# treangenlab/komb

Measured on AMD Instinct MI355X. Metric: peeled edges/sec (k-truss), higher is better.
Workload: dtype int32

## Files before the change

komb_amd/api.py:

```python
import ctypes
import os

import numpy as np

from . import _lib
from ._lib import KombOpts, KombStats, as_c, ptr


class KombError(RuntimeError):
    def __init__(self, code, msg):
        super().__init__(f"komb_accel error {code}: {msg}")
        self.code = code


def gen_hug_edges(nv, n_cliques, alpha=2.6, seed=42):
    lib = _lib.load()
    n_raw = lib.komb_gen_hug_edges(nv, n_cliques, alpha, seed, None)
    if n_raw < 0:
        raise ValueError("komb_gen_hug_edges: bad arguments")
    uv = np.empty((n_raw, 2), dtype=np.int64)
    got = lib.komb_gen_hug_edges(nv, n_cliques, alpha, seed, ptr(uv))
    assert got == n_raw
    return uv


FORWARD_ENV_OPTIONS = False
OPTION_NAMES = ("FINISH", "LOCAL_LIMIT", "LOCAL_ITEMS", "LOCAL_DENSITY", "LOCAL_DEFER_CHUNKS", "TAIL", "CORE_TAIL", "INDEX",
                "REC_CAP", "OWN_DENSE_CAP", "NO_OWN_DENSE", "NO_REC_SCRATCH", "NO_FIRST_QUEUE", "FULL_CAPS", "PREP_ROW_STAGE", "RETIRE_EVERY", "SHARD_ENGINE",
                "TRI_DEBUG", "POOL_DEBUG", "BUILD_DEBUG", "LOCAL_DEBUG", "TAIL_DEBUG", "COMP_SAMPLE", "COMM_SHORT", "COMM_HEAVY", "POISON")

SENTINEL_I32 = -0x5A5A5A5B


def _out_i32(n):
    return np.full(n, SENTINEL_I32, dtype=np.int32)


def _out_f64(n):
    return np.full(n, np.nan, dtype=np.float64)


class KombAccel:
    def __init__(self, device=0, verbosity=0, flags=0):
        self._lib = _lib.load()
        opts = KombOpts(device=device, verbosity=verbosity)
        opts.reserved[0] = flags
        self._ctx = self._lib.komb_create(ctypes.byref(opts))
        if not self._ctx:
            raise MemoryError("komb_create failed")
        self.device = device
        self.nv = -1
        self.ne = 0
        self._forwarded = {}

    def set_option(self, name, value):
        v = None if value is None else str(value).encode()
        self._check(self._lib.komb_set_option(self._ctx, name.encode(), v))

    def _sync_env_options(self):
        if not FORWARD_ENV_OPTIONS:
            return
        for name in OPTION_NAMES:
            v = os.environ.get("KOMB_" + name)
            if name == "INDEX" and os.environ.get("KOMB_TWO_PASS"):
                v = "two_pass"
            if name == "SHARD_ENGINE" and v is None:
                v = os.environ.get("KOMB_SHARD_PEEL")
            if self._forwarded.get(name) != v:
                self.set_option(name, v)
                self._forwarded[name] = v

    def close(self):
        if getattr(self, "_ctx", None):
            self._lib.komb_destroy(self._ctx)
            self._ctx = None

    def __del__(self):
        self.close()

    def __enter__(self):
        return self

    def __exit__(self, *a):
        self.close()

    def _check(self, rc):
        if rc != 0:
            raise KombError(rc, self._lib.komb_last_error(self._ctx).decode())

    def from_edges(self, nv, uv):
        uv = as_c(np.asarray(uv).reshape(-1, 2), np.int64)
        self._sync_env_options()
        self._check(self._lib.komb_graph_from_edges(self._ctx, nv, uv.shape[0], ptr(uv)))
        self._info()
        return self

    def from_csr(self, rowptr, col):
        rowptr = as_c(rowptr, np.int64)
        col = as_c(col, np.int32)
        self._sync_env_options()
        self._check(self._lib.komb_graph_from_csr(self._ctx, len(rowptr) - 1, ptr(rowptr), ptr(col)))
        self._info()
        return self

    def _info(self):
        nv, ne = ctypes.c_int64(), ctypes.c_int64()
        self._check(self._lib.komb_graph_info(self._ctx, ctypes.byref(nv), ctypes.byref(ne)))
        self.nv, self.ne = nv.value, ne.value

    def get_csr(self):
        rowptr = np.full(self.nv + 1, SENTINEL_I32, dtype=np.int64)
# ... 244 lines not shown
```

komb_amd/csrc/truss_prep.hip:

```cpp
#include "truss_line.h"

#include <algorithm>

namespace komb {

namespace {

constexpr uint32_t kPrepHeavy = 2048;
constexpr uint32_t kRowCap = 1024;
constexpr uint32_t kRowStage = 8192;
constexpr int kPW = kBlock / kWave;
constexpr int kPrepU = 4;

__global__ __launch_bounds__(kBlock) void k_prep_vertex(const uint32_t *__restrict__ rowptr, const int32_t *__restrict__ col, int64_t nv,
                                                        uint32_t *__restrict__ dkey, uint32_t *__restrict__ dval,
                                                        uint32_t *__restrict__ first_upper, uint32_t *__restrict__ upper_cnt)
{
    for (int64_t v = (int64_t)blockIdx.x * kBlock + threadIdx.x; v <= nv; v += (int64_t)gridDim.x * kBlock) {
        if (v == nv) { upper_cnt[v] = 0u; continue; }
        const uint32_t b = rowptr[v], e = rowptr[v + 1];
        dkey[v] = e - b;
        dval[v] = (uint32_t)v;
        uint32_t lo = b, hi = e;
        while (lo < hi) {
            const uint32_t mid = lo + ((hi - lo) >> 1);
            if (col[mid] < (int32_t)v) lo = mid + 1; else hi = mid;
        }
        first_upper[v] = lo;
        upper_cnt[v] = e - lo;
    }
}

__global__ __launch_bounds__(kBlock) void k_prep_invert(const uint32_t *__restrict__ sorted_ids, const uint32_t *__restrict__ sorted_deg,
                                                        const uint32_t *__restrict__ regbase, int64_t nv, int32_t *__restrict__ i2o, int32_t *__restrict__ o2i,
                                                        uint32_t *__restrict__ backcur, uint32_t *__restrict__ nlocal)
{
    for (int64_t i = (int64_t)blockIdx.x * kBlock + threadIdx.x; i < nv; i += (int64_t)gridDim.x * kBlock) {
        const uint32_t v = sorted_ids[i];
        i2o[i] = (int32_t)v;
        o2i[v] = (int32_t)i;
        const uint32_t r0 = regbase[i], d = sorted_deg[i];
        backcur[i] = r0 + d - 1u;
        if (d > kPrepHeavy) nlocal[v] = 0u;
    }
}

__device__ __forceinline__ int owner_of(const uint32_t *s_end, uint32_t it)
{
    int lo = 0;
#pragma unroll
    for (int st = kWave / 2; st > 0; st >>= 1) lo += (s_end[lo + st - 1] <= it) ? st : 0;
    return lo;
}

__global__ __launch_bounds__(kBlock) void k_prep_kept(const uint32_t *__restrict__ rowptr, const int32_t *__restrict__ col, int64_t nv,
                                                      const int32_t *__restrict__ o2i, const uint32_t *__restrict__ fu, const uint32_t *__restrict__ ebase,
                                                      const uint32_t *__restrict__ regbase,
                                                      uint2 *__restrict__ tmp, uint32_t *__restrict__ nlocal, uint32_t *__restrict__ backcur)
{
    __shared__ uint32_t sh_end[kPW][kWave], sh_beg[kPW][kWave], sh_a[kPW][kWave], sh_rp[kPW][kWave], sh_eb[kPW][kWave], sh_cnt[kPW][kWave];
    const int lane = lane_id(), w = (int)(threadIdx.x >> 6);
    uint32_t *s_end = sh_end[w], *s_beg = sh_beg[w], *s_a = sh_a[w], *s_rp = sh_rp[w], *s_eb = sh_eb[w], *s_cnt = sh_cnt[w];
    const int64_t gw = ((int64_t)blockIdx.x * kBlock + threadIdx.x) >> 6, nw = ((int64_t)gridDim.x * kBlock) >> 6;
    const int64_t ntasks = (nv + kWave - 1) / kWave;
    for (int64_t task = gw; task < ntasks; task += nw) {
        const int64_t v0 = task * kWave, v = v0 + lane;
        const bool has = v < nv;
        const uint32_t beg = has ? rowptr[v] : 0u, end = has ? rowptr[v + 1] : 0u, up = has ? fu[v] : 0u;
        const bool heavy = end - beg > kPrepHeavy;
        const uint32_t incl = wave_incl_scan(heavy ? 0u : end - up);
        const uint32_t total = (uint32_t)__shfl((int)incl, kWave - 1);
        __builtin_amdgcn_wave_barrier();
        s_end[lane] = incl;
        s_beg[lane] = up;
        const uint32_t av = has ? (uint32_t)o2i[v] : 0u;
        s_a[lane] = av;
        s_rp[lane] = has ? regbase[av] : 0u;
        s_eb[lane] = has ? ebase[v] : 0u;
        s_cnt[lane] = 0u;
        __builtin_amdgcn_wave_barrier();
        for (uint32_t it0 = 0; it0 < total; it0 += kWave * kPrepU) {
            int t[kPrepU];
            uint32_t rowstart[kPrepU], j[kPrepU], b[kPrepU];
            int32_t wv[kPrepU];
            bool on[kPrepU];
#pragma unroll
            for (int u = 0; u < kPrepU; ++u) {
                const uint32_t it = it0 + (uint32_t)(u * kWave + lane);
                on[u] = it < total;
                t[u] = on[u] ? owner_of(s_end, it) : 0;
                rowstart[u] = t[u] ? s_end[t[u] - 1] : 0u;
                j[u] = s_beg[t[u]] + (it - rowstart[u]);
            }
#pragma unroll
            for (int u = 0; u < kPrepU; ++u) wv[u] = on[u] ? col[j[u]] : 0;
#pragma unroll
            for (int u = 0; u < kPrepU; ++u) b[u] = on[u] ? (uint32_t)o2i[wv[u]] : 0u;
#pragma unroll
            for (int u = 0; u < kPrepU; ++u) {
                const uint32_t base = it0 + (uint32_t)(u * kWave), it = base + (uint32_t)lane;
                if (base >= total) break;
                const int tt = t[u];
                const uint32_t a = s_a[tt];
                const uint32_t k = s_eb[tt] + (it - rowstart[u]);
                const bool mine = on[u] && b[u] > a, theirs = on[u] && b[u] < a;
                if (theirs) tmp[atomicSub(&backcur[b[u]], 1u)] = make_uint2(a, k);
                const uint64_t K = __ballot(mine);
                const uint32_t f = rowstart[u] > base ? rowstart[u] - base : 0u;
                const uint32_t r = s_cnt[tt] + (uint32_t)__popcll(K & lanemask_lt() & ~((1ull << f) - 1ull));
                if (mine) tmp[(size_t)s_rp[tt] + r] = make_uint2(b[u], k);
                __builtin_amdgcn_wave_barrier();
                if (on[u] && (it + 1u == s_end[tt] || lane == kWave - 1)) s_cnt[tt] = r + (mine ? 1u : 0u);
                __builtin_amdgcn_wave_barrier();
            }
        }
        if (has && !heavy) nlocal[v] = s_cnt[lane];
        __builtin_amdgcn_wave_barrier();
    }
}

constexpr uint32_t kHeavyChunk = 256;
__global__ __launch_bounds__(kBlock) void k_prep_kept_heavy(const uint32_t *__restrict__ rowptr, const int32_t *__restrict__ col, int64_t nv,
                                                            const uint32_t *__restrict__ sorted_deg, const int32_t *__restrict__ i2o,
                                                            const int32_t *__restrict__ o2i, const uint32_t *__restrict__ fu, const uint32_t *__restrict__ ebase,
                                                            const uint32_t *__restrict__ regbase,
                                                            uint2 *__restrict__ tmp, uint32_t *__restrict__ nlocal, uint32_t *__restrict__ backcur)
{
    const int lane = lane_id();
    const uint32_t wi = (uint32_t)(((int64_t)blockIdx.x * kBlock + threadIdx.x) >> 6), W = (uint32_t)(((int64_t)gridDim.x * kBlock) >> 6);
    uint32_t cbase = 0;
    for (int64_t h0 = 0; h0 < nv; h0 += kWave) {
        const int64_t a = nv - 1 - h0 - lane;
        const uint32_t deg = a >= 0 ? sorted_deg[a] : 0u;
        const bool hv = deg > kPrepHeavy;
        const uint64_t HM = __ballot(hv);
        if (HM == 0) break;
        int32_t v = 0;
        uint32_t fuv = 0, eb = 0, reg = 0, end = 0;
        if (hv) { v = i2o[a]; fuv = fu[v]; eb = ebase[v]; reg = regbase[a]; end = rowptr[v] + deg; }
        const uint32_t nch = hv ? (end - fuv + kHeavyChunk - 1) / kHeavyChunk : 0u;
        uint32_t inc = nch;
#pragma unroll
        for (int d = 1; d < kWave; d <<= 1) { const uint32_t t = (uint32_t)__shfl_up((int)inc, d); if (lane >= d) inc += t; }
        const int nh = __popcll(HM);
        const uint32_t tot = (uint32_t)__shfl((int)inc, kWave - 1);
        for (uint32_t rel = (wi + W - (cbase % W)) % W; rel < tot; rel += W) {
            const int t = __popcll(__ballot(inc <= rel));
            const uint32_t c = rel - ((uint32_t)__shfl((int)inc, t) - (uint32_t)__shfl((int)nch, t));
            const int32_t rv = __shfl(v, t);
            const uint32_t ra = (uint32_t)(nv - 1 - h0 - t);
            const uint32_t r_fu = (uint32_t)__shfl((int)fuv, t), r_eb = (uint32_t)__shfl((int)eb, t), r_reg = (uint32_t)__shfl((int)reg, t), r_end = (uint32_t)__shfl((int)end, t);
            {
                const uint32_t j0 = r_fu + c * kHeavyChunk;
                constexpr int kU = (int)(kHeavyChunk / kWave);
                bool on[kU];
                int32_t wv[kU];
                uint32_t b[kU];
#pragma unroll
                for (int u = 0; u < kU; ++u) { const uint32_t j = j0 + (uint32_t)(u * kWave + lane); on[u] = j < r_end; wv[u] = on[u] ? col[j] : 0; }
#pragma unroll
                for (int u = 0; u < kU; ++u) b[u] = on[u] ? (uint32_t)o2i[wv[u]] : 0u;
#pragma unroll
                for (int u = 0; u < kU; ++u) {
                    const uint32_t k = r_eb + (j0 + (uint32_t)(u * kWave + lane) - r_fu);
                    const bool mine = on[u] && b[u] > ra, theirs = on[u] && b[u] < ra;
                    if (theirs) tmp[atomicSub(&backcur[b[u]], 1u)] = make_uint2(ra, k);
                    const uint64_t K = __ballot(mine);
                    if (K) {
                        const int lead = __ffsll((long long)K) - 1;
                        uint32_t base = 0;
                        if (lane == lead) base = atomicAdd(&nlocal[rv], (uint32_t)__popcll(K));
                        base = (uint32_t)__shfl((int)base, lead);
                        if (mine) tmp[(size_t)r_reg + base + (uint32_t)__popcll(K & lanemask_lt())] = make_uint2(b[u], k);
                    }
                }
            }
        }
        cbase += tot;
        if (nh < kWave) break;
    }
}

__global__ __launch_bounds__(kBlock) void k_prep_dplus(int64_t nv, const int32_t *__restrict__ i2o, const uint32_t *__restrict__ sorted_deg,
                                                       const uint32_t *__restrict__ regbase, const uint32_t *__restrict__ backcur,
                                                       const uint32_t *__restrict__ nlocal,
                                                       uint32_t *__restrict__ dplus_i, uint4 *__restrict__ where_i, unsigned long long *__restrict__ own_bound)
{
    unsigned long long ob = 0;
    for (int64_t a = (int64_t)blockIdx.x * kBlock + threadIdx.x; a < nv; a += (int64_t)gridDim.x * kBlock) {
        const uint32_t nl = nlocal[i2o[a]], bk = backcur[a] + 1u, reg = regbase[a];
        const unsigned long long d = nl + (reg + sorted_deg[a] - bk);
        dplus_i[a] = (uint32_t)d;
        where_i[a] = make_uint4(reg, nl, bk, 0u);
        ob += d ? d * (d - 1ull) : 0ull;
    }
    block_add_u64(ob, own_bound);
}

__global__ __launch_bounds__(kBlock) void k_prep_rows(const uint32_t *__restrict__ orow, int64_t nv, const uint4 *__restrict__ where_i,
                                                      const uint2 *__restrict__ tmp, int32_t *__restrict__ ocol,
                                                      uint32_t *__restrict__ e2k, uint4 *__restrict__ line)
{
    __shared__ int32_t sh_b[kPW][kRowCap];
    __shared__ uint32_t sh_kk[kPW][kRowCap];
    __shared__ unsigned long long sh_sig[kPW][kWave][kSigBlocks];
    __shared__ int32_t sh_piv[kPW][kWave][kPivots];
    __shared__ uint32_t sh_end[kPW][kWave], sh_rp[kPW][kWave], sh_ob[kPW][kWave], sh_nl[kPW][kWave], sh_bk[kPW][kWave];
    const int lane = lane_id(), w = (int)(threadIdx.x >> 6);
    int32_t *s_b = sh_b[w];
    uint32_t *s_kk = sh_kk[w], *s_end = sh_end[w], *s_rp = sh_rp[w], *s_ob = sh_ob[w], *s_nl = sh_nl[w], *s_bk = sh_bk[w];
    unsigned long long (*s_sig)[kSigBlocks] = sh_sig[w];
    int32_t (*s_piv)[kPivots] = sh_piv[w];
    const int64_t gw = ((int64_t)blockIdx.x * kBlock + threadIdx.x) >> 6, nw = ((int64_t)gridDim.x * kBlock) >> 6;
    const int64_t ntasks = (nv + kWave - 1) / kWave;
    for (int64_t task = gw; task < ntasks; task += nw) {
        const int64_t a0 = task * kWave, a = a0 + lane;
        const bool has = a < nv;
        const uint32_t ob = has ? orow[a] : 0u, d = has ? orow[a + 1] - ob : 0u;
        const bool big = d > kRowCap;
        const uint4 wh = has ? where_i[a] : make_uint4(0u, 0u, 0u, 0u);
        const uint32_t len = big ? 0u : d;
        __builtin_amdgcn_wave_barrier();
        s_rp[lane] = wh.x;
        s_nl[lane] = wh.y;
        s_bk[lane] = wh.z;
        s_ob[lane] = ob;
#pragma unroll
        for (int x = 0; x < kSigBlocks; ++x) s_sig[lane][x] = 0ull;
#pragma unroll
        for (int x = 0; x < kPivots; ++x) s_piv[lane][x] = 0x7FFFFFFF;
        for (int done = 0; done < kWave;) {
            const uint32_t incl = wave_incl_scan(lane >= done ? len : 0u);
            const int nfit = __popcll(__ballot(lane >= done && incl <= kRowCap));
            const int r1 = done + nfit;
            const uint32_t E = (uint32_t)__shfl((int)incl, r1 - 1);
            __builtin_amdgcn_wave_barrier();
            s_end[lane] = lane < done ? 0u : (lane < r1 ? incl : 0xFFFFFFFFu);
            __builtin_amdgcn_wave_barrier();
            for (uint32_t k = (uint32_t)lane; k < E; k += kWave) {
                const int t = owner_of(s_end, k);
                const uint32_t first = t ? s_end[t - 1] : 0u;
                const uint32_t idx = k - first, nl = s_nl[t];
                const uint2 ent = tmp[idx < nl ? (size_t)s_rp[t] + idx : (size_t)s_bk[t] + (idx - nl)];
                s_b[k] = (int32_t)ent.x; s_kk[k] = ent.y;
            }
            __builtin_amdgcn_wave_barrier();
            for (uint32_t k = (uint32_t)lane; k < E; k += kWave) {
                const int t = owner_of(s_end, k);
                const uint32_t first = t ? s_end[t - 1] : 0u, last = s_end[t];
                const int32_t mine = s_b[k];
                uint32_t rank = 0;
                for (uint32_t x = first; x < last; ++x) rank += s_b[x] < mine ? 1u : 0u;
                const uint32_t e = s_ob[t] + rank;
                ocol[e] = mine;
                e2k[e] = s_kk[k];
                uint32_t blk; unsigned long long mask;
                sig_slot(mine, blk, mask);
                atomicOr(&s_sig[t][blk], mask);
                const uint32_t seg = (last - first + (uint32_t)kPivots) / (uint32_t)(kPivots + 1);
                if (rank && rank % seg == 0u && rank / seg <= (uint32_t)kPivots) s_piv[t][rank / seg - 1u] = mine;
            }
            __builtin_amdgcn_wave_barrier();
            done = r1;
        }
        if (has && !big) {
            uint4 *L = line + 4 * a;
            const int32_t *pv = s_piv[lane];
            const unsigned long long *sg = s_sig[lane];
            L[0] = make_uint4(ob, d, (uint32_t)pv[0], (uint32_t)pv[1]);
            L[1] = make_uint4((uint32_t)pv[2], (uint32_t)pv[3], (uint32_t)pv[4], (uint32_t)pv[5]);
            L[2] = make_uint4((uint32_t)sg[0], (uint32_t)(sg[0] >> 32), (uint32_t)sg[1], (uint32_t)(sg[1] >> 32));
            L[3] = make_uint4((uint32_t)sg[2], (uint32_t)(sg[2] >> 32), (uint32_t)sg[3], (uint32_t)(sg[3] >> 32));
        }
        __builtin_amdgcn_wave_barrier();
// ... 142 lines not shown
            const uint32_t j = j0 + me;
            const int32_t wv = j < end ? col[j] : 0;
            const bool keep = j < end && mask[wv];
            const uint64_t K = __ballot(keep);
            uint32_t before = 0, all = (uint32_t)__popcll(K);
            if (WG) {
                __syncthreads();
                if (lane == 0) sh_wc[w] = all;
                __syncthreads();
                all = 0;
#pragma unroll
                for (int q = 0; q < kBlock / kWave; ++q) { const uint32_t c = sh_wc[q]; if (q < w) before += c; all += c; }
            }
            if (FILL && keep) sub_col[out0 + run + before + (uint32_t)__popcll(K & lanemask_lt())] = (int32_t)vnew[wv];
            run += all;
        }
        if (!FILL && me == 0) subdeg[x] = run;
    }
}

__global__ __launch_bounds__(kBlock) void k_edge_list(const uint32_t *__restrict__ rowptr, const int32_t *__restrict__ col, int64_t nv,
                                                      const uint32_t *__restrict__ fu, const uint32_t *__restrict__ ebase, const int32_t *__restrict__ vold,
                                                      int32_t *__restrict__ eu, int32_t *__restrict__ ev)
{
    const int lane = lane_id();
    const int64_t gw = ((int64_t)blockIdx.x * kBlock + threadIdx.x) >> 6, nw = ((int64_t)gridDim.x * kBlock) >> 6;
    for (int64_t v = gw; v < nv; v += nw) {
        const uint32_t j0 = fu[v], j1 = rowptr[v + 1], k0 = ebase[v];
        const int32_t uo = vold ? vold[v] : (int32_t)v;
        for (uint32_t j = j0 + (uint32_t)lane; j < j1; j += kWave) {
            const int32_t w = col[j];
            eu[k0 + (j - j0)] = uo;
            ev[k0 + (j - j0)] = vold ? vold[w] : w;
        }
    }
}

inline int id_bits(int64_t nv)
{
    int vb = 1;
    while (vb < 31 && (1ll << vb) < nv) ++vb;
    return vb;
}

template <class T> hipError_t pool_get(komb_ctx *ctx, T **out, size_t count)
{
    return ctx->pool.get((void **)out, (count ? count : 1) * sizeof(T));
}

}

void prep_free(komb_ctx *ctx, TrussPrep *p)
{
    void *all[] = {p->o2i, p->i2o, p->orow, p->ocol, p->osrc, p->e2k, p->vline, p->wtasks};
    for (void *q : all) ctx->pool.put(q);
    *p = TrussPrep{};
}

int prep_build(komb_ctx *ctx, const uint32_t *rowptr, const int32_t *col, int64_t nv, int64_t ns, TrussPrep *out)
{
    hipStream_t s = ctx->stream;
    const int64_t ne = ns / 2;
    Range r_all("truss: prepare");
    prep_free(ctx, out);
    TrussPrep P;
    P.nv = nv; P.ne = ne;
    struct Fail { komb_ctx *c; TrussPrep *p; bool armed = true; ~Fail() { if (armed) prep_free(c, p); } } fail{ctx, &P};
    EventSet evs;
    hipEvent_t ev[5] = {nullptr, nullptr, nullptr, nullptr, nullptr};
    for (auto &e : ev) KOMB_HIP(ctx, evs.make(&e));
    KOMB_HIP(ctx, hipEventRecord(ev[0], s));
    KOMB_HIP(ctx, pool_get(ctx, &P.o2i, (size_t)nv));
    KOMB_HIP(ctx, pool_get(ctx, &P.i2o, (size_t)nv));
    KOMB_HIP(ctx, pool_get(ctx, &P.orow, (size_t)nv + 1));
    KOMB_HIP(ctx, pool_get(ctx, &P.ocol, (size_t)ne + 8));
    KOMB_HIP(ctx, pool_get(ctx, &P.e2k, (size_t)ne));
    KOMB_HIP(ctx, pool_get(ctx, &P.vline, 4 * (size_t)nv));
    const size_t task_cap = 2 * (size_t)nv + (size_t)ne / kWave + 64;
    KOMB_HIP(ctx, pool_get(ctx, (uint2 **)&P.wtasks, task_cap));
    KOMB_HIP(ctx, hipMemsetAsync(P.ocol + ne, 0, 8 * sizeof(int32_t), s));

    DevBufs bufs(ctx);
    uint32_t *d_dk[2] = {nullptr, nullptr}, *d_dv[2] = {nullptr, nullptr}, *d_fu = nullptr, *d_uc = nullptr, *d_ebase = nullptr, *d_dplus = nullptr;
    uint32_t *d_nlocal = nullptr, *d_backcur = nullptr, *d_regbase = nullptr;
    uint4 *d_where = nullptr;
    uint32_t *d_tcnt = nullptr, *d_hlist = nullptr, *d_words = nullptr;
    unsigned long long *d_acc = nullptr;
    uint2 *d_tmp = nullptr;
    for (int i = 0; i < 2; ++i) { KOMB_HIP(ctx, bufs.alloc(&d_dk[i], (size_t)nv)); KOMB_HIP(ctx, bufs.alloc(&d_dv[i], (size_t)nv)); }
    KOMB_HIP(ctx, bufs.alloc(&d_fu, (size_t)nv + 1));
    KOMB_HIP(ctx, bufs.alloc(&d_uc, (size_t)nv + 1));
    KOMB_HIP(ctx, bufs.alloc(&d_ebase, (size_t)nv + 1));
    KOMB_HIP(ctx, bufs.alloc(&d_dplus, (size_t)nv + 1));
    KOMB_HIP(ctx, bufs.alloc(&d_nlocal, (size_t)nv));
    KOMB_HIP(ctx, bufs.alloc(&d_where, (size_t)nv));
    KOMB_HIP(ctx, bufs.alloc(&d_regbase, (size_t)nv + 1));
    KOMB_HIP(ctx, bufs.alloc(&d_backcur, (size_t)nv));
    KOMB_HIP(ctx, bufs.alloc(&d_tcnt, (size_t)nv + 1));
    const uint32_t hcap = (uint32_t)(ne / kRowCap + 64);
    KOMB_HIP(ctx, bufs.alloc(&d_hlist, (size_t)hcap));
    KOMB_HIP(ctx, bufs.alloc(&d_words, 4));
    KOMB_HIP(ctx, bufs.alloc(&d_acc, 8));
    KOMB_HIP(ctx, bufs.alloc(&d_tmp, (size_t)ns));
    KOMB_HIP(ctx, hipMemsetAsync(d_words, 0, 4 * sizeof(uint32_t), s));
    KOMB_HIP(ctx, hipMemsetAsync(d_acc, 0, 8 * sizeof(unsigned long long), s));
    KOMB_HIP(ctx, hipMemsetAsync(d_dplus + nv, 0, sizeof(uint32_t), s));

    const int gv = grid_for(nv + 1);
    const int gwave = grid_for((nv + kWave - 1) / kWave, kPW, 256 * 8);
    k_prep_vertex<<<gv, kBlock, 0, s>>>(rowptr, col, nv, d_dk[0], d_dv[0], d_fu, d_uc);
    uint32_t *sk = d_dk[0], *sv = d_dv[0];
    if (nv > 0) {
        KOMB_TRY(prim_sort_pairs_u32_u32(ctx, d_dk[0], d_dk[1], d_dv[0], d_dv[1], nv, id_bits(nv), &sk, &sv));
        KOMB_TRY(prim_exclusive_sum_u32(ctx, sk, d_regbase, nv));
        k_prep_invert<<<grid_for(nv), kBlock, 0, s>>>(sv, sk, d_regbase, nv, P.i2o, P.o2i, d_backcur, d_nlocal);
    }
    KOMB_TRY(prim_exclusive_sum_u32(ctx, d_uc, d_ebase, nv + 1));
    KOMB_HIP(ctx, hipEventRecord(ev[1], s));
    if (nv > 0) {
        k_prep_kept<<<gwave, kBlock, 0, s>>>(rowptr, col, nv, P.o2i, d_fu, d_ebase, d_regbase, d_tmp, d_nlocal, d_backcur);
        k_prep_kept_heavy<<<256 * 4, kBlock, 0, s>>>(rowptr, col, nv, sk, P.i2o, P.o2i, d_fu, d_ebase, d_regbase, d_tmp, d_nlocal, d_backcur);
        k_prep_dplus<<<grid_for(nv), kBlock, 0, s>>>(nv, P.i2o, sk, d_regbase, d_backcur, d_nlocal, d_dplus, d_where, d_acc);
    }
    KOMB_TRY(prim_exclusive_sum_u32(ctx, d_dplus, P.orow, nv + 1));
    KOMB_HIP(ctx, hipEventRecord(ev[2], s));
    const int group = (int)std::max<int64_t>(1, std::min<int64_t>(kWedgeV, nv / (256 * KOMB_WEDGE_EU * kTriWaves * 4)));
    k_task_count<<<gv, kBlock, 0, s>>>(P.orow, nv, group, d_tcnt, d_hlist, d_words, hcap);
    if (nv > 0) {
        k_prep_rows<<<gwave, kBlock, 0, s>>>(P.orow, nv, d_where, d_tmp, P.ocol, P.e2k, P.vline);
        uint32_t stage_cap = kRowStage;
        if (const char *e = ctx_opt(ctx, "PREP_ROW_STAGE")) stage_cap = std::min<uint32_t>(kRowStage, (uint32_t)strtoul(e, nullptr, 10));
        k_prep_rows_heavy<<<1024, kBlock, 0, s>>>(d_hlist, d_words, P.orow, d_where, d_tmp, P.ocol, P.e2k, P.vline, stage_cap);
    }
    KOMB_HIP(ctx, hipEventRecord(ev[3], s));
    KOMB_TRY(prim_exclusive_sum_u32(ctx, d_tcnt, d_tcnt, nv + 1));
    if (nv > 0) k_task_fill<<<grid_for(nv), kBlock, 0, s>>>(d_tcnt, nv, group, (uint2 *)P.wtasks);
    k_prep_flags<<<1, 64, 0, s>>>(d_tcnt, nv, d_words, d_acc, P.orow, d_acc + 1);
    KOMB_HIP(ctx, hipEventRecord(ev[4], s));
    unsigned long long h[4] = {0, 0, 0, 0};
    KOMB_HIP(ctx, d2h(ctx, h, d_acc + 1, sizeof(h)));
    float ms = 0.f, part[4] = {0.f, 0.f, 0.f, 0.f};
    (void)hipEventElapsedTime(&ms, ev[0], ev[4]);
    for (int i = 0; i < 4; ++i) (void)hipEventElapsedTime(&part[i], ev[i], ev[i + 1]);
    for (int i = 0; i < 4; ++i) P.ms_part[i] = (double)part[i];
    if (h[2] != (unsigned long long)ne) KOMB_FAIL(ctx, KOMB_ERR_DEVICE, "k-truss preparation: %llu oriented slots for %lld edges", h[2], (long long)ne);
    if (h[3] > hcap) KOMB_FAIL(ctx, KOMB_ERR_DEVICE, "k-truss preparation: %llu oriented rows beyond %u slots, room for %u", h[3], kRowCap, hcap);
    if (h[0] > task_cap) KOMB_FAIL(ctx, KOMB_ERR_DEVICE, "k-truss preparation: %llu tasks, room for %zu", h[0], task_cap);
    P.n_wtasks = (int64_t)h[0];
    P.own_bound = (int64_t)h[1];
    P.ms = (double)ms;
    P.valid = true;
    fail.armed = false;
    *out = P;
    return KOMB_OK;
}

namespace {
__global__ __launch_bounds__(kBlock) void k_prep_sources(const uint32_t *__restrict__ orow, int64_t nv, int32_t *__restrict__ osrc)
{
    const int lane = lane_id();
    const int64_t gw = ((int64_t)blockIdx.x * kBlock + threadIdx.x) >> 6, nw = ((int64_t)gridDim.x * kBlock) >> 6;
    for (int64_t a = gw; a < nv; a += nw)
        for (uint32_t e = orow[a] + (uint32_t)lane, e1 = orow[a + 1]; e < e1; e += kWave) osrc[e] = (int32_t)a;
}
}

int prep_sources(komb_ctx *ctx, TrussPrep *p)
{
    if (p->osrc || !p->valid) return KOMB_OK;
    KOMB_HIP(ctx, ctx->pool.get((void **)&p->osrc, (size_t)(p->ne ? p->ne : 1) * sizeof(int32_t)));
    if (p->nv > 0) k_prep_sources<<<grid_for(p->nv, kPW, 256 * 8), kBlock, 0, ctx->stream>>>(p->orow, p->nv, p->osrc);
    KOMB_HIP(ctx, hipGetLastError());
    return KOMB_OK;
}

int prep_ensure(komb_ctx *ctx)
{
    if (ctx->prep.valid) return KOMB_OK;
    return prep_build(ctx, ctx->d_o_rowptr, ctx->d_o_col, ctx->nv, 2 * ctx->ne, &ctx->prep);
}

int graph_moments(komb_ctx *ctx, int64_t out[5])
{
    KOMB_TRY(prep_ensure(ctx));
    KOMB_TRY(prep_sources(ctx, &ctx->prep));
    const TrussPrep &P = ctx->prep;
    unsigned long long *d_mom = nullptr, h[5] = {0, 0, 0, 0, 0};
    DevBufs bufs(ctx);
    KOMB_HIP(ctx, bufs.alloc(&d_mom, 5));
    KOMB_HIP(ctx, hipMemsetAsync(d_mom, 0, 5 * sizeof(unsigned long long), ctx->stream));
    k_graph_moments<<<1024, kBlock, 0, ctx->stream>>>(ctx->d_o_rowptr, P.nv, P.i2o, P.osrc, P.ocol, P.ne, P.orow, d_mom);
    KOMB_HIP(ctx, d2h(ctx, h, d_mom, sizeof(h)));
    for (int i = 0; i < 5; ++i) out[i] = (int64_t)h[i];
    return KOMB_OK;
}

void induced_free(komb_ctx *ctx, InducedCsr *g)
{
    ctx->pool.put(g->rowptr); ctx->pool.put(g->col); ctx->pool.put(g->vold);
    *g = InducedCsr{};
}

int induce_csr(komb_ctx *ctx, const uint8_t *vmask_host, InducedCsr *out)
{
    hipStream_t s = ctx->stream;
    const int64_t nv = ctx->nv;
    InducedCsr G;
    struct Fail { komb_ctx *c; InducedCsr *g; bool armed = true; ~Fail() { if (armed) induced_free(c, g); } } fail{ctx, &G};
    DevBufs bufs(ctx);
    uint8_t *d_mask = nullptr;
    uint32_t *d_flag = nullptr, *d_vnew = nullptr, *d_subdeg = nullptr;
    KOMB_HIP(ctx, bufs.alloc(&d_mask, (size_t)nv));
    KOMB_HIP(ctx, bufs.alloc(&d_flag, (size_t)nv + 1));
    KOMB_HIP(ctx, bufs.alloc(&d_vnew, (size_t)nv + 1));
    KOMB_HIP(ctx, hipMemcpyAsync(d_mask, vmask_host, (size_t)nv, hipMemcpyHostToDevice, s));
    k_mask_flags<<<grid_for(nv + 1), kBlock, 0, s>>>(d_mask, nv, d_flag);
    KOMB_TRY(prim_exclusive_sum_u32(ctx, d_flag, d_vnew, nv + 1));
    uint32_t nk = 0;
    KOMB_HIP(ctx, d2h(ctx, &nk, d_vnew + nv, sizeof(uint32_t)));
    G.nv = (int64_t)nk;
    KOMB_HIP(ctx, pool_get(ctx, &G.vold, (size_t)nk));
    KOMB_HIP(ctx, pool_get(ctx, &G.rowptr, (size_t)nk + 1));
    KOMB_HIP(ctx, bufs.alloc(&d_subdeg, (size_t)nk + 1));
    uint32_t n_slots = 0;
    if (nk > 0) {
        uint32_t *d_hlist = nullptr, *d_hcount = nullptr;
        KOMB_HIP(ctx, bufs.alloc(&d_hlist, (size_t)(2 * ctx->ne) / kPrepHeavy + 64));
        KOMB_HIP(ctx, bufs.alloc(&d_hcount, 1));
        KOMB_HIP(ctx, hipMemsetAsync(d_hcount, 0, sizeof(uint32_t), s));
        k_mask_list<<<grid_for(nv), kBlock, 0, s>>>(d_mask, d_vnew, nv, G.vold);
        KOMB_HIP(ctx, hipMemsetAsync(d_subdeg + nk, 0, sizeof(uint32_t), s));
        const int gw = grid_for(nk, kPW, 256 * 8);
        k_induce<false, false><<<gw, kBlock, 0, s>>>(ctx->d_o_rowptr, ctx->d_o_col, d_mask, d_vnew, G.vold, nk, d_subdeg, nullptr, nullptr, d_hlist, d_hcount);
        k_induce<false, true><<<1024, kBlock, 0, s>>>(ctx->d_o_rowptr, ctx->d_o_col, d_mask, d_vnew, G.vold, nk, d_subdeg, nullptr, nullptr, d_hlist, d_hcount);
        KOMB_TRY(prim_exclusive_sum_u32(ctx, d_subdeg, G.rowptr, (int64_t)nk + 1));
        KOMB_HIP(ctx, d2h(ctx, &n_slots, G.rowptr + nk, sizeof(uint32_t)));
        KOMB_HIP(ctx, pool_get(ctx, &G.col, (size_t)n_slots));
        if (n_slots > 0) {
            k_induce<true, false><<<gw, kBlock, 0, s>>>(ctx->d_o_rowptr, ctx->d_o_col, d_mask, d_vnew, G.vold, nk, nullptr, G.rowptr, G.col, d_hlist, d_hcount);
            k_induce<true, true><<<1024, kBlock, 0, s>>>(ctx->d_o_rowptr, ctx->d_o_col, d_mask, d_vnew, G.vold, nk, nullptr, G.rowptr, G.col, d_hlist, d_hcount);
        }
    } else {
        KOMB_HIP(ctx, hipMemsetAsync(G.rowptr, 0, sizeof(uint32_t), s));
        KOMB_HIP(ctx, pool_get(ctx, &G.col, 1));
    }
    G.ns = (int64_t)n_slots;
    KOMB_HIP(ctx, hipStreamSynchronize(s));
    fail.armed = false;
    *out = G;
    return KOMB_OK;
}

int edge_list(komb_ctx *ctx, const uint32_t *rowptr, const int32_t *col, int64_t nv, const int32_t *vold, int32_t *eu, int32_t *ev)
{
    hipStream_t s = ctx->stream;
    DevBufs bufs(ctx);
    uint32_t *d_dk = nullptr, *d_dv = nullptr, *d_fu = nullptr, *d_uc = nullptr, *d_ebase = nullptr;
    KOMB_HIP(ctx, bufs.alloc(&d_dk, (size_t)nv)); KOMB_HIP(ctx, bufs.alloc(&d_dv, (size_t)nv));
    KOMB_HIP(ctx, bufs.alloc(&d_fu, (size_t)nv + 1)); KOMB_HIP(ctx, bufs.alloc(&d_uc, (size_t)nv + 1)); KOMB_HIP(ctx, bufs.alloc(&d_ebase, (size_t)nv + 1));
    k_prep_vertex<<<grid_for(nv + 1), kBlock, 0, s>>>(rowptr, col, nv, d_dk, d_dv, d_fu, d_uc);
    KOMB_TRY(prim_exclusive_sum_u32(ctx, d_uc, d_ebase, nv + 1));
    if (nv > 0) k_edge_list<<<grid_for(nv, kPW, 256 * 8), kBlock, 0, s>>>(rowptr, col, nv, d_fu, d_ebase, vold, eu, ev);
    KOMB_HIP(ctx, hipStreamSynchronize(s));
    return KOMB_OK;
}

}
```

Before: 4.058 billion.

## Sort only vertices above a degree cap and rank the rest by bitmap

```diff
diff --git a/komb_amd/api.py b/komb_amd/api.py
--- a/komb_amd/api.py
+++ b/komb_amd/api.py
@@ -26,7 +26,7 @@
 
 FORWARD_ENV_OPTIONS = False
 OPTION_NAMES = ("FINISH", "LOCAL_LIMIT", "LOCAL_ITEMS", "LOCAL_DENSITY", "LOCAL_DEFER_CHUNKS", "TAIL", "CORE_TAIL", "INDEX",
-                "REC_CAP", "OWN_DENSE_CAP", "NO_OWN_DENSE", "NO_REC_SCRATCH", "NO_FIRST_QUEUE", "FULL_CAPS", "PREP_ROW_STAGE", "RETIRE_EVERY", "SHARD_ENGINE",
+                "REC_CAP", "OWN_DENSE_CAP", "NO_OWN_DENSE", "NO_REC_SCRATCH", "NO_FIRST_QUEUE", "FULL_CAPS", "PREP_ROW_STAGE", "PREP_LIGHT_CAP", "RETIRE_EVERY", "SHARD_ENGINE",
                 "TRI_DEBUG", "POOL_DEBUG", "BUILD_DEBUG", "LOCAL_DEBUG", "TAIL_DEBUG", "COMP_SAMPLE", "COMM_SHORT", "COMM_HEAVY", "POISON")
 
 SENTINEL_I32 = -0x5A5A5A5B
diff --git a/komb_amd/csrc/truss_prep.hip b/komb_amd/csrc/truss_prep.hip
--- a/komb_amd/csrc/truss_prep.hip
+++ b/komb_amd/csrc/truss_prep.hip
@@ -12,36 +12,79 @@
 constexpr int kPW = kBlock / kWave;
 constexpr int kPrepU = 4;
 
-__global__ __launch_bounds__(kBlock) void k_prep_vertex(const uint32_t *__restrict__ rowptr, const int32_t *__restrict__ col, int64_t nv,
-                                                        uint32_t *__restrict__ dkey, uint32_t *__restrict__ dval,
+constexpr uint32_t kPrepLightCap = 0;
+
+__device__ __forceinline__ uint32_t class_id(uint2 hw, uint32_t v, const uint32_t *__restrict__ hrank, uint32_t n_light)
+{
+    const uint32_t bit = 1u << (v & 31u), below = hw.y + (uint32_t)__popc(hw.x & (bit - 1u));
+    return (hw.x & bit) ? n_light + hrank[below] : v - below;
+}
+
+__global__ __launch_bounds__(kBlock) void k_prep_vertex(const uint32_t *__restrict__ rowptr, const int32_t *__restrict__ col, int64_t nv, uint32_t cap,
+                                                        uint2 *__restrict__ hb, uint32_t *__restrict__ hcnt,
+                                                        uint32_t *__restrict__ plist, uint32_t *__restrict__ pcount,
                                                         uint32_t *__restrict__ first_upper, uint32_t *__restrict__ upper_cnt)
 {
-    for (int64_t v = (int64_t)blockIdx.x * kBlock + threadIdx.x; v <= nv; v += (int64_t)gridDim.x * kBlock) {
-        if (v == nv) { upper_cnt[v] = 0u; continue; }
-        const uint32_t b = rowptr[v], e = rowptr[v + 1];
-        dkey[v] = e - b;
-        dval[v] = (uint32_t)v;
-        uint32_t lo = b, hi = e;
-        while (lo < hi) {
-            const uint32_t mid = lo + ((hi - lo) >> 1);
-            if (col[mid] < (int32_t)v) lo = mid + 1; else hi = mid;
-        }
-        first_upper[v] = lo;
-        upper_cnt[v] = e - lo;
-    }
-}
-
-__global__ __launch_bounds__(kBlock) void k_prep_invert(const uint32_t *__restrict__ sorted_ids, const uint32_t *__restrict__ sorted_deg,
-                                                        const uint32_t *__restrict__ regbase, int64_t nv, int32_t *__restrict__ i2o, int32_t *__restrict__ o2i,
+    const int lane = lane_id();
+    for (int64_t v0 = (int64_t)blockIdx.x * kBlock + threadIdx.x - lane; v0 <= nv; v0 += (int64_t)gridDim.x * kBlock) {
+        const int64_t v = v0 + lane;
+        uint32_t deg = 0;
+        if (v < nv) {
+            const uint32_t b = rowptr[v], e = rowptr[v + 1];
+            deg = e - b;
+            uint32_t lo = b, hi = e;
+            while (lo < hi) {
+                const uint32_t mid = lo + ((hi - lo) >> 1);
+                if (col[mid] < (int32_t)v) lo = mid + 1; else hi = mid;
+            }
+            first_upper[v] = lo;
+            upper_cnt[v] = e - lo;
+            if (plist && deg > kPrepHeavy) plist[atomicAdd(pcount, 1u)] = (uint32_t)v;
+        } else if (v == nv) upper_cnt[v] = 0u;
+        const uint64_t H = __ballot(deg > cap);
+        if (hb && v < nv && (lane & 31) == 0) {
+            const uint32_t m = (uint32_t)(H >> lane);
+            hb[v >> 5].x = m;
+            hcnt[v >> 5] = (uint32_t)__popc(m);
+        }
+    }
+}
+
+__global__ __launch_bounds__(kBlock) void k_prep_classes(const uint32_t *__restrict__ rowptr, int64_t nv, uint2 *__restrict__ hb, const uint32_t *__restrict__ hpre,
+                                                         int32_t *__restrict__ i2o, int32_t *__restrict__ o2i, uint32_t *__restrict__ ideg,
+                                                         uint32_t *__restrict__ hkey, uint32_t *__restrict__ hval)
+{
+    for (int64_t v = (int64_t)blockIdx.x * kBlock + threadIdx.x; v < nv; v += (int64_t)gridDim.x * kBlock) {
+        const uint32_t m = hb[v >> 5].x, pre = hpre[v >> 5], bit = 1u << (v & 31);
+        const uint32_t below = pre + (uint32_t)__popc(m & (bit - 1u)), deg = rowptr[v + 1] - rowptr[v];
+        if ((v & 31) == 0) hb[v >> 5].y = pre;
+        if (m & bit) { hkey[below] = deg; hval[below] = (uint32_t)v; }
+        else { const uint32_t a = (uint32_t)v - below; i2o[a] = (int32_t)v; o2i[v] = (int32_t)a; ideg[a] = deg; }
+    }
+}
+
+__global__ __launch_bounds__(kBlock) void k_prep_heavy_ids(const uint32_t *__restrict__ sorted_deg, const uint32_t *__restrict__ sorted_ids, int64_t n_heavy,
+                                                           uint32_t n_light, const uint2 *__restrict__ hb, uint32_t *__restrict__ hrank,
+                                                           int32_t *__restrict__ i2o, int32_t *__restrict__ o2i, uint32_t *__restrict__ ideg)
+{
+    for (int64_t r = (int64_t)blockIdx.x * kBlock + threadIdx.x; r < n_heavy; r += (int64_t)gridDim.x * kBlock) {
+        const uint32_t v = sorted_ids[r], a = n_light + (uint32_t)r;
+        const uint2 hw = hb[v >> 5];
+        hrank[hw.y + (uint32_t)__popc(hw.x & ((1u << (v & 31u)) - 1u))] = (uint32_t)r;
+        i2o[a] = (int32_t)v;
+        o2i[v] = (int32_t)a;
+        ideg[a] = sorted_deg[r];
+    }
+}
+
+__global__ __launch_bounds__(kBlock) void k_prep_invert(const int32_t *__restrict__ i2o, const uint32_t *__restrict__ ideg,
+                                                        const uint32_t *__restrict__ regbase, int64_t nv,
                                                         uint32_t *__restrict__ backcur, uint32_t *__restrict__ nlocal)
 {
     for (int64_t i = (int64_t)blockIdx.x * kBlock + threadIdx.x; i < nv; i += (int64_t)gridDim.x * kBlock) {
-        const uint32_t v = sorted_ids[i];
-        i2o[i] = (int32_t)v;
-        o2i[v] = (int32_t)i;
-        const uint32_t r0 = regbase[i], d = sorted_deg[i];
+        const uint32_t r0 = regbase[i], d = ideg[i];
         backcur[i] = r0 + d - 1u;
-        if (d > kPrepHeavy) nlocal[v] = 0u;
+        if (d > kPrepHeavy) nlocal[i2o[i]] = 0u;
     }
 }
 
@@ -53,8 +96,10 @@
     return lo;
 }
 
+template <bool TABLE>
 __global__ __launch_bounds__(kBlock) void k_prep_kept(const uint32_t *__restrict__ rowptr, const int32_t *__restrict__ col, int64_t nv,
-                                                      const int32_t *__restrict__ o2i, const uint32_t *__restrict__ fu, const uint32_t *__restrict__ ebase,
+                                                      const int32_t *__restrict__ o2i, const uint2 *__restrict__ hb, const uint32_t *__restrict__ hrank, uint32_t n_light,
+                                                      const uint32_t *__restrict__ fu, const uint32_t *__restrict__ ebase,
                                                       const uint32_t *__restrict__ regbase,
                                                       uint2 *__restrict__ tmp, uint32_t *__restrict__ nlocal, uint32_t *__restrict__ backcur)
 {
@@ -73,7 +118,7 @@
         __builtin_amdgcn_wave_barrier();
         s_end[lane] = incl;
         s_beg[lane] = up;
-        const uint32_t av = has ? (uint32_t)o2i[v] : 0u;
+        const uint32_t av = !has ? 0u : TABLE ? class_id(hb[v >> 5], (uint32_t)v, hrank, n_light) : (uint32_t)o2i[v];
         s_a[lane] = av;
         s_rp[lane] = has ? regbase[av] : 0u;
         s_eb[lane] = has ? ebase[v] : 0u;
@@ -83,6 +128,7 @@
             int t[kPrepU];
             uint32_t rowstart[kPrepU], j[kPrepU], b[kPrepU];
             int32_t wv[kPrepU];
+            uint2 hw[kPrepU];
             bool on[kPrepU];
 #pragma unroll
             for (int u = 0; u < kPrepU; ++u) {
@@ -95,7 +141,9 @@
 #pragma unroll
             for (int u = 0; u < kPrepU; ++u) wv[u] = on[u] ? col[j[u]] : 0;
 #pragma unroll
-            for (int u = 0; u < kPrepU; ++u) b[u] = on[u] ? (uint32_t)o2i[wv[u]] : 0u;
+            for (int u = 0; u < kPrepU; ++u) hw[u] = TABLE && on[u] ? hb[wv[u] >> 5] : make_uint2(0u, 0u);
+#pragma unroll
+            for (int u = 0; u < kPrepU; ++u) b[u] = !on[u] ? 0u : TABLE ? class_id(hw[u], (uint32_t)wv[u], hrank, n_light) : (uint32_t)o2i[wv[u]];
 #pragma unroll
             for (int u = 0; u < kPrepU; ++u) {
                 const uint32_t base = it0 + (uint32_t)(u * kWave), it = base + (uint32_t)lane;
@@ -120,46 +168,51 @@
 }
 
 constexpr uint32_t kHeavyChunk = 256;
-__global__ __launch_bounds__(kBlock) void k_prep_kept_heavy(const uint32_t *__restrict__ rowptr, const int32_t *__restrict__ col, int64_t nv,
-                                                            const uint32_t *__restrict__ sorted_deg, const int32_t *__restrict__ i2o,
-                                                            const int32_t *__restrict__ o2i, const uint32_t *__restrict__ fu, const uint32_t *__restrict__ ebase,
+template <bool TABLE>
+__global__ __launch_bounds__(kBlock) void k_prep_kept_heavy(const uint32_t *__restrict__ rowptr, const int32_t *__restrict__ col,
+                                                            const uint32_t *__restrict__ plist, const uint32_t *__restrict__ pcount,
+                                                            const int32_t *__restrict__ o2i, const uint2 *__restrict__ hb, const uint32_t *__restrict__ hrank, uint32_t n_light,
+                                                            const uint32_t *__restrict__ fu, const uint32_t *__restrict__ ebase,
                                                             const uint32_t *__restrict__ regbase,
                                                             uint2 *__restrict__ tmp, uint32_t *__restrict__ nlocal, uint32_t *__restrict__ backcur)
 {
     const int lane = lane_id();
     const uint32_t wi = (uint32_t)(((int64_t)blockIdx.x * kBlock + threadIdx.x) >> 6), W = (uint32_t)(((int64_t)gridDim.x * kBlock) >> 6);
+    const uint32_t np = *pcount;
     uint32_t cbase = 0;
-    for (int64_t h0 = 0; h0 < nv; h0 += kWave) {
-        const int64_t a = nv - 1 - h0 - lane;
-        const uint32_t deg = a >= 0 ? sorted_deg[a] : 0u;
-        const bool hv = deg > kPrepHeavy;
-        const uint64_t HM = __ballot(hv);
-        if (HM == 0) break;
+    for (uint32_t h0 = 0; h0 < np; h0 += kWave) {
+        const bool hv = h0 + (uint32_t)lane < np;
         int32_t v = 0;
-        uint32_t fuv = 0, eb = 0, reg = 0, end = 0;
-        if (hv) { v = i2o[a]; fuv = fu[v]; eb = ebase[v]; reg = regbase[a]; end = rowptr[v] + deg; }
+        uint32_t a = 0, fuv = 0, eb = 0, reg = 0, end = 0;
+        if (hv) {
+            v = (int32_t)plist[h0 + (uint32_t)lane];
+            a = (uint32_t)o2i[v];
+            fuv = fu[v]; eb = ebase[v]; reg = regbase[a]; end = rowptr[v + 1];
+        }
         const uint32_t nch = hv ? (end - fuv + kHeavyChunk - 1) / kHeavyChunk : 0u;
         uint32_t inc = nch;
 #pragma unroll
         for (int d = 1; d < kWave; d <<= 1) { const uint32_t t = (uint32_t)__shfl_up((int)inc, d); if (lane >= d) inc += t; }
-        const int nh = __popcll(HM);
         const uint32_t tot = (uint32_t)__shfl((int)inc, kWave - 1);
         for (uint32_t rel = (wi + W - (cbase % W)) % W; rel < tot; rel += W) {
             const int t = __popcll(__ballot(inc <= rel));
             const uint32_t c = rel - ((uint32_t)__shfl((int)inc, t) - (uint32_t)__shfl((int)nch, t));
             const int32_t rv = __shfl(v, t);
-            const uint32_t ra = (uint32_t)(nv - 1 - h0 - t);
+            const uint32_t ra = (uint32_t)__shfl((int)a, t);
             const uint32_t r_fu = (uint32_t)__shfl((int)fuv, t), r_eb = (uint32_t)__shfl((int)eb, t), r_reg = (uint32_t)__shfl((int)reg, t), r_end = (uint32_t)__shfl((int)end, t);
             {
                 const uint32_t j0 = r_fu + c * kHeavyChunk;
                 constexpr int kU = (int)(kHeavyChunk / kWave);
                 bool on[kU];
                 int32_t wv[kU];
+                uint2 hw[kU];
                 uint32_t b[kU];
 #pragma unroll
                 for (int u = 0; u < kU; ++u) { const uint32_t j = j0 + (uint32_t)(u * kWave + lane); on[u] = j < r_end; wv[u] = on[u] ? col[j] : 0; }
 #pragma unroll
-                for (int u = 0; u < kU; ++u) b[u] = on[u] ? (uint32_t)o2i[wv[u]] : 0u;
+                for (int u = 0; u < kU; ++u) hw[u] = TABLE && on[u] ? hb[wv[u] >> 5] : make_uint2(0u, 0u);
+#pragma unroll
+                for (int u = 0; u < kU; ++u) b[u] = !on[u] ? 0u : TABLE ? class_id(hw[u], (uint32_t)wv[u], hrank, n_light) : (uint32_t)o2i[wv[u]];
 #pragma unroll
                 for (int u = 0; u < kU; ++u) {
                     const uint32_t k = r_eb + (j0 + (uint32_t)(u * kWave + lane) - r_fu);
@@ -177,11 +230,10 @@
             }
         }
         cbase += tot;
-        if (nh < kWave) break;
-    }
-}
-
-__global__ __launch_bounds__(kBlock) void k_prep_dplus(int64_t nv, const int32_t *__restrict__ i2o, const uint32_t *__restrict__ sorted_deg,
+    }
+}
+
+__global__ __launch_bounds__(kBlock) void k_prep_dplus(int64_t nv, const int32_t *__restrict__ i2o, const uint32_t *__restrict__ ideg,
                                                        const uint32_t *__restrict__ regbase, const uint32_t *__restrict__ backcur,
                                                        const uint32_t *__restrict__ nlocal,
                                                        uint32_t *__restrict__ dplus_i, uint4 *__restrict__ where_i, unsigned long long *__restrict__ own_bound)
@@ -189,7 +241,7 @@
     unsigned long long ob = 0;
     for (int64_t a = (int64_t)blockIdx.x * kBlock + threadIdx.x; a < nv; a += (int64_t)gridDim.x * kBlock) {
         const uint32_t nl = nlocal[i2o[a]], bk = backcur[a] + 1u, reg = regbase[a];
-        const unsigned long long d = nl + (reg + sorted_deg[a] - bk);
+        const unsigned long long d = nl + (reg + ideg[a] - bk);
         dplus_i[a] = (uint32_t)d;
         where_i[a] = make_uint4(reg, nl, bk, 0u);
         ob += d ? d * (d - 1ull) : 0ull;
@@ -498,12 +550,19 @@
 
     DevBufs bufs(ctx);
     uint32_t *d_dk[2] = {nullptr, nullptr}, *d_dv[2] = {nullptr, nullptr}, *d_fu = nullptr, *d_uc = nullptr, *d_ebase = nullptr, *d_dplus = nullptr;
+    uint2 *d_hb = nullptr;
+    uint32_t *d_hcnt = nullptr, *d_hpre = nullptr, *d_hrank = nullptr, *d_ideg = nullptr, *d_plist = nullptr;
     uint32_t *d_nlocal = nullptr, *d_backcur = nullptr, *d_regbase = nullptr;
     uint4 *d_where = nullptr;
     uint32_t *d_tcnt = nullptr, *d_hlist = nullptr, *d_words = nullptr;
     unsigned long long *d_acc = nullptr;
     uint2 *d_tmp = nullptr;
-    for (int i = 0; i < 2; ++i) { KOMB_HIP(ctx, bufs.alloc(&d_dk[i], (size_t)nv)); KOMB_HIP(ctx, bufs.alloc(&d_dv[i], (size_t)nv)); }
+    const int64_t nwords = (nv + 31) / 32;
+    KOMB_HIP(ctx, bufs.alloc(&d_hb, (size_t)nwords));
+    KOMB_HIP(ctx, bufs.alloc(&d_hcnt, (size_t)nwords + 1));
+    KOMB_HIP(ctx, bufs.alloc(&d_hpre, (size_t)nwords + 1));
+    KOMB_HIP(ctx, bufs.alloc(&d_ideg, (size_t)nv));
+    KOMB_HIP(ctx, bufs.alloc(&d_plist, (size_t)ns / kPrepHeavy + 64));
     KOMB_HIP(ctx, bufs.alloc(&d_fu, (size_t)nv + 1));
     KOMB_HIP(ctx, bufs.alloc(&d_uc, (size_t)nv + 1));
     KOMB_HIP(ctx, bufs.alloc(&d_ebase, (size_t)nv + 1));
@@ -524,19 +583,39 @@
 
     const int gv = grid_for(nv + 1);
     const int gwave = grid_for((nv + kWave - 1) / kWave, kPW, 256 * 8);
-    k_prep_vertex<<<gv, kBlock, 0, s>>>(rowptr, col, nv, d_dk[0], d_dv[0], d_fu, d_uc);
-    uint32_t *sk = d_dk[0], *sv = d_dv[0];
+    uint32_t cap = kPrepLightCap;
+    if (const char *e = ctx_opt(ctx, "PREP_LIGHT_CAP")) cap = (uint32_t)std::min<unsigned long long>(strtoull(e, nullptr, 10), 0xFFFFFFFFull);
+    KOMB_HIP(ctx, hipMemsetAsync(d_hcnt + nwords, 0, sizeof(uint32_t), s));
+    k_prep_vertex<<<gv, kBlock, 0, s>>>(rowptr, col, nv, cap, d_hb, d_hcnt, d_plist, d_words + 1, d_fu, d_uc);
+    uint32_t n_heavy = 0;
     if (nv > 0) {
-        KOMB_TRY(prim_sort_pairs_u32_u32(ctx, d_dk[0], d_dk[1], d_dv[0], d_dv[1], nv, id_bits(nv), &sk, &sv));
-        KOMB_TRY(prim_exclusive_sum_u32(ctx, sk, d_regbase, nv));
-        k_prep_invert<<<grid_for(nv), kBlock, 0, s>>>(sv, sk, d_regbase, nv, P.i2o, P.o2i, d_backcur, d_nlocal);
-    }
+        KOMB_TRY(prim_exclusive_sum_u32(ctx, d_hcnt, d_hpre, nwords + 1));
+        d_dk[0] = (uint32_t *)d_tmp; d_dv[0] = d_dk[0] + ns;
+        k_prep_classes<<<grid_for(nv), kBlock, 0, s>>>(rowptr, nv, d_hb, d_hpre, P.i2o, P.o2i, d_ideg, d_dk[0], d_dv[0]);
+        KOMB_HIP(ctx, d2h(ctx, &n_heavy, d_hpre + nwords, sizeof(uint32_t)));
+        if ((int64_t)n_heavy > std::min(nv, ns)) KOMB_FAIL(ctx, KOMB_ERR_DEVICE, "k-truss preparation: %u heavy vertices of %lld", n_heavy, (long long)nv);
+        KOMB_HIP(ctx, bufs.alloc(&d_dk[1], (size_t)n_heavy)); KOMB_HIP(ctx, bufs.alloc(&d_dv[1], (size_t)n_heavy));
+        KOMB_HIP(ctx, bufs.alloc(&d_hrank, (size_t)n_heavy));
+        if (n_heavy > 0) {
+            uint32_t *sk = nullptr, *sv = nullptr;
+            KOMB_TRY(prim_sort_pairs_u32_u32(ctx, d_dk[0], d_dk[1], d_dv[0], d_dv[1], (int64_t)n_heavy, id_bits(nv), &sk, &sv));
+            k_prep_heavy_ids<<<grid_for((int64_t)n_heavy), kBlock, 0, s>>>(sk, sv, (int64_t)n_heavy, (uint32_t)nv - n_heavy, d_hb, d_hrank, P.i2o, P.o2i, d_ideg);
+        }
+        KOMB_TRY(prim_exclusive_sum_u32(ctx, d_ideg, d_regbase, nv));
+        k_prep_invert<<<grid_for(nv), kBlock, 0, s>>>(P.i2o, d_ideg, d_regbase, nv, d_backcur, d_nlocal);
+    }
+    const uint32_t n_light = (uint32_t)nv - n_heavy;
     KOMB_TRY(prim_exclusive_sum_u32(ctx, d_uc, d_ebase, nv + 1));
     KOMB_HIP(ctx, hipEventRecord(ev[1], s));
     if (nv > 0) {
-        k_prep_kept<<<gwave, kBlock, 0, s>>>(rowptr, col, nv, P.o2i, d_fu, d_ebase, d_regbase, d_tmp, d_nlocal, d_backcur);
-        k_prep_kept_heavy<<<256 * 4, kBlock, 0, s>>>(rowptr, col, nv, sk, P.i2o, P.o2i, d_fu, d_ebase, d_regbase, d_tmp, d_nlocal, d_backcur);
-        k_prep_dplus<<<grid_for(nv), kBlock, 0, s>>>(nv, P.i2o, sk, d_regbase, d_backcur, d_nlocal, d_dplus, d_where, d_acc);
+        if (cap > 0) {
+            k_prep_kept<true><<<gwave, kBlock, 0, s>>>(rowptr, col, nv, P.o2i, d_hb, d_hrank, n_light, d_fu, d_ebase, d_regbase, d_tmp, d_nlocal, d_backcur);
+            k_prep_kept_heavy<true><<<256 * 4, kBlock, 0, s>>>(rowptr, col, d_plist, d_words + 1, P.o2i, d_hb, d_hrank, n_light, d_fu, d_ebase, d_regbase, d_tmp, d_nlocal, d_backcur);
+        } else {
+            k_prep_kept<false><<<gwave, kBlock, 0, s>>>(rowptr, col, nv, P.o2i, d_hb, d_hrank, n_light, d_fu, d_ebase, d_regbase, d_tmp, d_nlocal, d_backcur);
+            k_prep_kept_heavy<false><<<256 * 4, kBlock, 0, s>>>(rowptr, col, d_plist, d_words + 1, P.o2i, d_hb, d_hrank, n_light, d_fu, d_ebase, d_regbase, d_tmp, d_nlocal, d_backcur);
+        }
+        k_prep_dplus<<<grid_for(nv), kBlock, 0, s>>>(nv, P.i2o, d_ideg, d_regbase, d_backcur, d_nlocal, d_dplus, d_where, d_acc);
     }
     KOMB_TRY(prim_exclusive_sum_u32(ctx, d_dplus, P.orow, nv + 1));
     KOMB_HIP(ctx, hipEventRecord(ev[2], s));
@@ -671,10 +750,9 @@
 {
     hipStream_t s = ctx->stream;
     DevBufs bufs(ctx);
-    uint32_t *d_dk = nullptr, *d_dv = nullptr, *d_fu = nullptr, *d_uc = nullptr, *d_ebase = nullptr;
-    KOMB_HIP(ctx, bufs.alloc(&d_dk, (size_t)nv)); KOMB_HIP(ctx, bufs.alloc(&d_dv, (size_t)nv));
+    uint32_t *d_fu = nullptr, *d_uc = nullptr, *d_ebase = nullptr;
     KOMB_HIP(ctx, bufs.alloc(&d_fu, (size_t)nv + 1)); KOMB_HIP(ctx, bufs.alloc(&d_uc, (size_t)nv + 1)); KOMB_HIP(ctx, bufs.alloc(&d_ebase, (size_t)nv + 1));
-    k_prep_vertex<<<grid_for(nv + 1), kBlock, 0, s>>>(rowptr, col, nv, d_dk, d_dv, d_fu, d_uc);
+    k_prep_vertex<<<grid_for(nv + 1), kBlock, 0, s>>>(rowptr, col, nv, 0u, nullptr, nullptr, nullptr, nullptr, d_fu, d_uc);
     KOMB_TRY(prim_exclusive_sum_u32(ctx, d_uc, d_ebase, nv + 1));
     if (nv > 0) k_edge_list<<<grid_for(nv, kPW, 256 * 8), kBlock, 0, s>>>(rowptr, col, nv, d_fu, d_ebase, vold, eu, ev);
     KOMB_HIP(ctx, hipStreamSynchronize(s));
```

Result: no change. 4.042 billion (median of 2 runs) (-0.4%).
